# mandt-lab/PSLD

Hardware: AMD Instinct MI355X
Metric: train images/sec, CIFAR-10 PSLD (6ch 32x32) NCSN++ HSM step (higher is better)
Workload: dtype f32

## Files before the change

### include/psld_hip.h

```cpp
#ifndef PSLD_HIP_H
#define PSLD_HIP_H

#if defined(__HIP__) || defined(__HIPCC__)
#include <hip/hip_runtime_api.h>
#else
typedef struct ihipStream_t* hipStream_t;
#endif

#ifdef __cplusplus
extern "C" {
#endif


#define PSLD_ABI_VERSION 14
#define PSLD_COEFF_STRIDE 12

int psld_version(void);
const char* psld_last_error(void);

#define PSLD_MATH_F32 0
#define PSLD_MATH_BF16X6 1
#define PSLD_MATH_BF16X3 2
int psld_set_math_mode(int mode);
int psld_get_math_mode(void);
// ... 100 lines not shown
                           hipStream_t stream);
int psld_pack_frag_batch_x3(const long long* table_dev, int entries, long long total_items, hipStream_t stream);
int psld_gemm_split_x3_f32(const float* a1, int k1, const float* a2, int k2, int m, const void* bfrag, int n,
                           float* y, int ldy, const psld_epilogue_t* epi, hipStream_t stream);

int psld_attn_fwd_split_supported(int hw, int c);
int psld_attn_fwd_split_f32(const float* q, const float* k, const float* v, int ld, int batch, int hw, int c, float scale,
                            float* o, int ldo, float* p, hipStream_t stream);

int psld_conv3x3_wgrad_split_supported(int cout, int cin, int batch, int h, int w);
int psld_conv3x3_wgrad_split_cout_tile(int cout);
int psld_conv3x3_wgrad_split_f32(const float* dy, int lddy, int cout, const float* x, int cin,
                                 const float* x2, int cin2, int batch, int h, int w, float* slabs,
                                 int cin_total, int col0, int nsplit, hipStream_t stream);
int psld_conv3x3_wgrad_xlimb_f32(const float* dy, int lddy, int cout, const void* x_limb, int cin,
                                 const void* x2_limb, int cin2, int batch, int h, int w, float* slabs,
                                 int cin_total, int col0, int nsplit, hipStream_t stream);
int psld_conv3x3_wgrad_wino_supported(int cout, int cin, int cin2, int batch, int h, int w);
int psld_conv3x3_wgrad_wino_nsplit(int cout, int cin_total, int batch, int h, int w);
long long psld_conv3x3_wgrad_wino_ws_bytes(int cout, int cin_total, int nsplit);
int psld_conv3x3_wgrad_wino_f32(const float* dy, int lddy, int cout, const float* x, int cin, const float* x2, int cin2,
                                int batch, int h, int w, float* slabs, int nsplit, float* dw_oihw, int accumulate,
                                float alpha, hipStream_t stream);
int psld_gemm_tn_split_supported(int m, int n, int k);
int psld_gemm_tn_split_f32(int m, int n, int k, const float* a, int lda, const float* b, int ldb,
                           const float* b2, int ldb2, int n2, float* slabs, int ldc, int nsplit, hipStream_t stream);

int psld_bgemm_split_supported(int ta, int tb, int m, int n, int k);
int psld_bgemm_split_f32(int ta, int tb, int m, int n, int k, const float* a, int lda, long long stride_a,
                         const float* b, int ldb, long long stride_b, float* c, int ldc, long long stride_c,
                         int batch, float alpha, hipStream_t stream);

int psld_conv2d_wgrad_nhwc_f32(const float* dy, int lddy, int cout,
                               const float* x, int cin, int batch, int ih, int iw,
                               int kh, int kw, int stride, int pad, int oh, int ow,
                               float* slabs, int cin_total, int col0, int nsplit,
                               hipStream_t stream);

int psld_reduce_slabs_f32(const float* slabs, int nsplit, long long n, float* out,
                          int layout, int cout, int taps, int cin, float alpha, hipStream_t stream);

int psld_pack_oihw_to_ohwi_f32(const float* w, float* out, int cout, int cin, int taps, hipStream_t stream);
int psld_pack_oihw_to_dgrad_f32(const float* w, float* out, int cout, int cin, int taps, hipStream_t stream);

int psld_nchw_to_nhwc_f32(const float* x, float* y, int batch, int c, int hw, hipStream_t stream);
int psld_nhwc_to_nchw_f32(const float* x, float* y, int batch, int c, int hw, hipStream_t stream);
// ... 164 lines not shown
```

### psld_amd/_lib.py

```python
from __future__ import annotations

import ctypes as C
import os

_HERE = os.path.dirname(os.path.abspath(__file__))
LIB_PATH = os.environ.get("PSLD_HIP_LIB") or os.path.join(_HERE, "libpsld_hip.so")

c_f32p = C.c_void_p
c_f64p = C.c_void_p
c_stream = C.c_void_p
c_ll = C.c_longlong


class Epilogue(C.Structure):
    _fields_ = [
        ("alpha", C.c_float),
        ("bias", C.c_void_p),
        ("rowbias", C.c_void_p),
        ("ld_rowbias", C.c_int),
        ("rows_per_img", C.c_int),
        ("residual", C.c_void_p),
        ("ld_residual", C.c_int),
        ("residual_stride_batch", C.c_longlong),
        ("out_scale", C.c_float),
# ... 3 lines not shown
        ("gn_fine", C.c_int),
    ]


class SdeParams(C.Structure):
    _fields_ = [
        ("beta_0", C.c_double), ("beta_1", C.c_double), ("nu", C.c_double), ("gamma", C.c_double),
        ("m_inv", C.c_double), ("numerical_eps", C.c_double), ("decomp_lower", C.c_int),
    ]


class EmCoeffs(C.Structure):
    _fields_ = [
        ("beta", C.c_double), ("m_inv", C.c_double), ("gamma", C.c_double), ("nu", C.c_double),
        ("m", C.c_double),
        ("c11", C.c_float), ("c12", C.c_float), ("c21", C.c_float), ("c22", C.c_float),
        ("dt", C.c_double), ("score_mode", C.c_int), ("probability_flow", C.c_int),
    ]


class SscsCoeffs(C.Structure):
    _fields_ = [(n, C.c_double) for n in ("a_xx", "a_xm", "a_mx", "a_mm", "c11", "c12", "c21", "c22")]


I, F, D, LL, P = C.c_int, C.c_float, C.c_double, C.c_longlong, C.c_void_p
EP = C.POINTER(Epilogue)

ABI_VERSION = 14

SIGNATURES = {
    "psld_version": (I, []),
    "psld_last_error": (C.c_char_p, []),
    "psld_set_math_mode": (I, [I]),
    "psld_get_math_mode": (I, []),
    "psld_set_gn_bwd_kernel": (I, [I]),
    "psld_get_gn_bwd_kernel": (I, []),
    "psld_gemm_f32": (I, [I, I, I, I, I, P, I, LL, P, I, LL, P, I, LL, I, EP, P]),
    "psld_gemm_tn_splitk_f32": (I, [I, I, I, P, I, P, I, P, I, P]),
    "psld_conv2d_nhwc_f32": (I, [P, I, P, I, I, I, I, P, I, I, I, I, I, I, I, I, P, I, EP, P]),
    "psld_conv2d_workspace_bytes": (LL, [I, I, I, I]),
    "psld_conv2d_nhwc_ws_f32": (I, [P, I, P, I, I, I, I, P, I, I, I, I, I, I, I, I, P, I, EP, P, LL, P]),
    "psld_conv2d_wgrad_nhwc_f32": (I, [P, I, I, P, I, I, I, I, I, I, I, I, I, I, P, I, I, I, P]),
    "psld_conv3x3_frag_bytes": (LL, [I, I]),
    "psld_conv3x3_split_supported": (I, [I, I, I, I, I, I]),
    "psld_pack_conv3x3_frag": (I, [P, P, I, I, I, P]),
    "psld_pack_frag_batch": (I, [P, I, LL, P]),
# ... 18 lines not shown
    "psld_conv3x3_wino_gn_x3_f32": (I, [P, I, P, P, P, I, P, P, I, I, I, I, P, I, P, I, EP, P, LL, P]),
    "psld_gn_apply_limb_nhwc": (I, [P, P, P, P, I, I, I, I, F, C.c_ulonglong, P, P]),
    "psld_limb_bytes": (LL, [LL, I]),
    "psld_f32_to_limb": (I, [P, LL, I, P, P]),
    "psld_limb_to_f32": (I, [P, LL, I, P, P]),
    "psld_conv3x3_limb_f32": (I, [P, I, P, I, I, I, I, P, I, P, I, EP, P, LL, P]),
    "psld_gemm_frag_bytes": (LL, [I, I]),
    "psld_gemm_split_supported": (I, [I, I, I, I]),
    "psld_pack_gemm_frag": (I, [P, P, I, I, LL, LL, P]),
    "psld_gemm_split_f32": (I, [P, I, P, I, I, P, I, P, I, EP, P, LL, P]),
    "psld_gemm_frag_bytes_x3": (LL, [I, I]),
    "psld_gemm_split_x3_supported": (I, [I, I, I, I]),
    "psld_pack_gemm_frag_x3": (I, [P, P, I, I, LL, LL, P]),
    "psld_pack_frag_batch_x3": (I, [P, I, LL, P]),
    "psld_gemm_split_x3_f32": (I, [P, I, P, I, I, P, I, P, I, EP, P]),
    "psld_conv3x3_wgrad_split_supported": (I, [I, I, I, I, I]),
    "psld_conv3x3_wgrad_split_cout_tile": (I, [I]),
    "psld_conv3x3_wgrad_split_f32": (I, [P, I, I, P, I, P, I, I, I, I, P, I, I, I, P]),
    "psld_conv3x3_wgrad_xlimb_f32": (I, [P, I, I, P, I, P, I, I, I, I, P, I, I, I, P]),
    "psld_conv3x3_wgrad_wino_supported": (I, [I, I, I, I, I, I]),
    "psld_conv3x3_wgrad_wino_nsplit": (I, [I, I, I, I, I]),
    "psld_conv3x3_wgrad_wino_ws_bytes": (LL, [I, I, I]),
    "psld_conv3x3_wgrad_wino_f32": (I, [P, I, I, P, I, P, I, I, I, I, P, I, P, I, F, P]),
    "psld_gemm_tn_split_supported": (I, [I, I, I]),
    "psld_gemm_tn_split_f32": (I, [I, I, I, P, I, P, I, P, I, I, P, I, I, P]),
    "psld_bgemm_split_supported": (I, [I, I, I, I, I]),
    "psld_bgemm_split_f32": (I, [I, I, I, I, I, P, I, LL, P, I, LL, P, I, LL, I, F, P]),
    "psld_reduce_slabs_f32": (I, [P, I, LL, P, I, I, I, I, F, P]),
    "psld_pack_oihw_to_ohwi_f32": (I, [P, P, I, I, I, P]),
    "psld_pack_oihw_to_dgrad_f32": (I, [P, P, I, I, I, P]),
    "psld_nchw_to_nhwc_f32": (I, [P, P, I, I, I, P]),
    "psld_nhwc_to_nchw_f32": (I, [P, P, I, I, I, P]),
    "psld_gn_workspace_bytes": (LL, [I, I, I, I]),
    "psld_gn_stats_nhwc_f32": (I, [P, I, I, I, I, F, P, P, P, P, P, P, P, P]),
    "psld_gn_stats_from_partials_f32": (I, [P, I, I, I, I, I, F, P, P, P, P, P, P, P]),
    "psld_gn_apply_nhwc_f32": (I, [P, P, P, P, I, I, I, I, F, C.c_ulonglong, P, P]),
    "psld_gn_bwd_nhwc_f32": (I, [P, P, P, P, P, P, I, I, I, I, I, F, C.c_ulonglong, P, P, I, P, F, P, P, I, P, P]),
    "psld_gn_bwd_colsum_supported": (I, [I, I, I, I]),
    "psld_gn_bwd_team_rows": (I, [I, I, I, I]),
    "psld_gn_bwd_team_sync_bytes": (LL, []),
    "psld_gn_bwd_team_f32": (I, [P, P, P, P, P, P, I, I, I, I, I, F, C.c_ulonglong, P, P, I, P, F, P, P, I, P, P]),
    "psld_param_reduce2_f32": (I, [P, P, I, I, I, P, P, F, P]),
    "psld_param_reduce_batch_f32": (I, [P, I, I, P]),
    "psld_reduce_slabs_batch_units": (I, [LL, I, I, I]),
    "psld_reduce_slabs_batch_f32": (I, [P, I, LL, P]),
    "psld_upfirdn2d_f32": (I, [P, P, I, I, I, I, P, I, I, I, I, I, I, I, I, I, I, I, I, P]),
# ... 108 lines not shown
```

### psld_amd/csrc/wgrad_wino.hip

```cpp
#include "limb.h"
#include "psld_hip.h"
#include "tile_shared.h"

namespace {

typedef __attribute__((ext_vector_type(4))) short s16x4;
__device__ __forceinline__ u32x2 lds_tr16(const unsigned char* p) {
    const s16x4 v = __builtin_amdgcn_ds_read_tr16_b64_v4i16(
        (__attribute__((address_space(3))) s16x4*)(__attribute__((address_space(3))) void*)(p));
    return __builtin_bit_cast(u32x2, v);
}

constexpr int WW_CI = 128;
constexpr int WW_RSB = WW_CI * 2 + 32;
constexpr int WW_BLIMB = 32 * WW_RSB;
template <int CO>
struct WWGeom {
    static constexpr int RSA = CO * 2 + 32;
    static constexpr int ALIMB = 32 * RSA;
    static constexpr int IMG = 3 * (ALIMB + WW_BLIMB);
    static constexpr size_t LDS = 2 * (size_t)IMG;
    static constexpr int NY = CO / 32;
    static constexpr int CB = CO / 32;
};
// ... 42 lines not shown

template <int ABL = 0>
__device__ __forceinline__ void ww_store(unsigned char* d, int limb_stride, const f32x4& v) {
    unsigned h0, m0, l0, h1, m1, l1;
    if constexpr ((ABL & 1) != 0) {
        h0 = m0 = l0 = __float_as_uint(v[0]) ^ __float_as_uint(v[1]);
        h1 = m1 = l1 = __float_as_uint(v[2]) ^ __float_as_uint(v[3]);
    } else {
        ww_split3(v[0], v[1], h0, m0, l0);
        ww_split3(v[2], v[3], h1, m1, l1);
    }
    *reinterpret_cast<u32x2*>(d) = u32x2{h0, h1};
    *reinterpret_cast<u32x2*>(d + limb_stride) = u32x2{m0, m1};
    *reinterpret_cast<u32x2*>(d + 2 * limb_stride) = u32x2{l0, l1};
}

__device__ __forceinline__ f32x4 bload(const __amdgpu_buffer_rsrc_t& r, unsigned off) {
    return __builtin_bit_cast(f32x4, __builtin_amdgcn_raw_buffer_load_b128(r, off, 0, 0));
}
__device__ __forceinline__ __amdgpu_buffer_rsrc_t brsrc(const float* p) {
    return __builtin_amdgcn_make_buffer_rsrc(const_cast<float*>(p), 0, 0x7fffffff, 0x00020000);
}

template <int ABL = 0, int CO = 256, bool TAIL = false>
__global__ void __launch_bounds__(512) wwgrad_ws_kernel(const WWgradArgs a) {
    using G = WWGeom<CO>;
    constexpr int WW_CO = CO, WW_RSA = G::RSA, WW_ALIMB = G::ALIMB, WW_IMG = G::IMG, NY = G::NY, CB = G::CB;
    extern __shared__ __attribute__((aligned(16))) unsigned char smem[];
    const int tid = threadIdx.x;
    const int lane = tid & 63, wave = __builtin_amdgcn_readfirstlane(tid >> 6);

    const int units = 16 * a.cin_tiles * a.cout_tiles;
    const int vid = xcd_remap(blockIdx.x, gridDim.x);
    const int split = vid / units;
    int rest = vid - split * units;
    int pos = rest & 15;
    if constexpr (ABL != 0) {
        if (a.pos_override >= 0) pos = a.pos_override;
    }
    rest >>= 4;
    const int ci_tile = rest % a.cin_tiles, co_tile = rest / a.cin_tiles;
    const int pi = pos >> 2, pj = pos & 3;
    const int co0 = co_tile * WW_CO, ci_out = ci_tile * WW_CI;
    const int kt_beg = split * a.ktiles_per_split;
    const int nkt = min(a.ktiles_per_split, a.ktiles - kt_beg);

    if (wave >= 4) {
        const bool second = ci_out >= a.cin;
        const float* xsrc = second ? a.x2 : a.x;
        const int xc = second ? a.cin2 : a.cin;
        const int ci0 = second ? ci_out - a.cin : ci_out;
        const int pt = tid & 255;
        int xr1, xr2, xc1, xc2, yr1, ynr, yc1, ync;
        float xsr, xsc, ysr, ysc;
        x_combo(pi, xr1, xr2, xsr);
        x_combo(pj, xc1, xc2, xsc);
// ... 203 lines not shown
                for (int u = 0; u < 6; ++u)
#pragma unroll
                    for (int nb = 0; nb < 4; ++nb)
                        acc[cb][nb] = __builtin_amdgcn_mfma_f32_16x16x32_bf16(
                            __builtin_bit_cast(bf16x8, fa[cb & 1][PA[u]]), __builtin_bit_cast(bf16x8, fb[nb][PB[u]]), acc[cb][nb], 0, 0, 0);
            }
        }
        __syncthreads();
    }

    float* S = a.slabs + ((long long)split * 16 + pos) * a.cout * a.cin_total;
#pragma unroll
    for (int cb = 0; cb < CB; ++cb)
#pragma unroll
        for (int nb = 0; nb < 4; ++nb)
#pragma unroll
            for (int v = 0; v < 4; ++v) {
                const int co = co0 + wr * (CO / 2) + cb * 16 + 4 * g + v;
                if (!TAIL || (co < a.cout && ci_out + wc * 64 + nb * 16 + i16 < a.cin_total))
                    S[(long long)co * a.cin_total + ci_out + wc * 64 + nb * 16 + i16] = acc[cb][nb][v];
            }
}

__global__ void __launch_bounds__(64) wwgrad_reduce_kernel(const float* __restrict__ slabs, int nsplit, long long n, float* __restrict__ dw,
                                                           int accumulate, float alpha) {
    const long long idx = (long long)blockIdx.x * 64 + threadIdx.x;
    if (idx >= n) return;
    float m[16];
#pragma unroll
    for (int p = 0; p < 16; ++p) m[p] = 0.f;
    const float* src = slabs + idx;
    for (int sp = 0; sp < nsplit; ++sp) {
        float v[16];
#pragma unroll
        for (int p = 0; p < 16; ++p) v[p] = __builtin_nontemporal_load(src + ((long long)sp * 16 + p) * n);
#pragma unroll
        for (int p = 0; p < 16; ++p) m[p] += v[p];
    }
    float t[4][3];
#pragma unroll
    for (int i = 0; i < 4; ++i) {
        const float h = 0.5f * (m[4 * i + 1] + m[4 * i + 2]), d = 0.5f * (m[4 * i + 1] - m[4 * i + 2]);
        t[i][0] = m[4 * i] + h;
        t[i][1] = d;
        t[i][2] = h - m[4 * i + 3];
    }
    float o[9];
#pragma unroll
    for (int kx = 0; kx < 3; ++kx) {
        const float h = 0.5f * (t[1][kx] + t[2][kx]), d = 0.5f * (t[1][kx] - t[2][kx]);
        o[kx] = t[0][kx] + h;
        o[3 + kx] = d;
        o[6 + kx] = h - t[3][kx];
    }
    float* out = dw + idx * 9;
#pragma unroll
    for (int e = 0; e < 9; ++e) out[e] = accumulate ? out[e] + alpha * o[e] : alpha * o[e];
}

inline int ww_co_tile(int cout) { return cout % 256 ? 128 : 256; }

int ilog2(int v) {
    int l = 0;
    while ((1 << l) < v) ++l;
    return l;
}

}

static bool ww_width_ok(int c) { return c >= 128 && c % 32 == 0; }

extern "C" int psld_conv3x3_wgrad_wino_supported(int cout, int cin, int cin2, int batch, int h, int w) {
    if (batch <= 0 || cin2 < 0 || !ww_width_ok(cout) || !ww_width_ok(cin) || (cin2 && (cin % WW_CI || !ww_width_ok(cin2)))) return 0;
    if (h != w || !(w == 8 || w == 16 || w == 32 || w == 64 || w == 128)) return 0;
    return ((long long)batch * h * w / 4) % 32 == 0;
}

extern "C" int psld_conv3x3_wgrad_wino_nsplit(int cout, int cin_total, int batch, int h, int w) {
    if (!ww_width_ok(cout) || !ww_width_ok(cin_total)) return 0;
    const int units = 16 * (int)cdiv(cout, ww_co_tile(cout)) * (int)cdiv(cin_total, WW_CI);
    const long long ktiles = (long long)batch * h * w / 4 / 32;
    static int cus[PSLD_MAX_DEVICES] = {};
    int& n = cus[psld_device_slot()];
    if (n == 0) {
        int dev = 0;
        if (hipGetDevice(&dev) != hipSuccess || hipDeviceGetAttribute(&n, hipDeviceAttributeMultiprocessorCount, dev) != hipSuccess || n <= 0) n = 256;
    }
    int ns = n / units;
    if (ns < 1) ns = 1;
    if (ns > ktiles) ns = (int)ktiles;
    const long long per = (ktiles + ns - 1) / ns;
    return (int)((ktiles + per - 1) / per);
}

extern "C" long long psld_conv3x3_wgrad_wino_ws_bytes(int cout, int cin_total, int nsplit) {
    return (long long)nsplit * 16 * cout * cin_total * 4;
}

extern "C" int psld_conv3x3_wgrad_wino_f32(const float* dy, int lddy, int cout, const float* x, int cin, const float* x2, int cin2,
                                           int batch, int h, int w, float* slabs, int nsplit, float* dw_oihw, int accumulate,
                                           float alpha, hipStream_t stream) {
    PSLD_CHECK_ARG(dy && x && slabs && dw_oihw && nsplit >= 1 && (cin2 == 0 || x2), "psld_conv3x3_wgrad_wino_f32: bad args");
    PSLD_CHECK_ARG(psld_conv3x3_wgrad_wino_supported(cout, cin, cin2, batch, h, w),
                   "psld_conv3x3_wgrad_wino_f32: unsupported shape cout=%d cin=%d+%d B=%d %dx%d", cout, cin, cin2, batch, h, w);
    PSLD_CHECK_ARG(aligned16(dy) && aligned16(x) && (cin2 == 0 || aligned16(x2)) && lddy % 4 == 0 && lddy >= cout,
                   "psld_conv3x3_wgrad_wino_f32: unaligned operand");
    const long long ktiles = (long long)batch * h * w / 4 / 32;
    const long long per_split = (ktiles + nsplit - 1) / nsplit;
    PSLD_CHECK_ARG((ktiles + per_split - 1) / per_split == nsplit, "psld_conv3x3_wgrad_wino_f32: %d splits of %lld K tiles leave empty slabs", nsplit, ktiles);
    WWgradArgs a{};
    a.dy = dy; a.lddy = lddy; a.x = x; a.cin = cin; a.x2 = x2; a.cin2 = cin2;
    a.H = h; a.W = w;
    const int tw = w / 2 < 32 ? w / 2 : 32;
    a.lg_tw = ilog2(tw); a.tw_mask = tw - 1; a.th_mask = h / 2 - 1;
    a.rows_per_kt = 32 >> a.lg_tw;
    a.lg_kpr = ilog2(w / 2 / tw); a.kpr_mask = w / 2 / tw - 1;
    const int co_tile = ww_co_tile(cout);
    a.cout_tiles = (int)cdiv(cout, co_tile); a.cin_tiles = (int)cdiv(cin + cin2, WW_CI);
    const bool tail = cout % co_tile || (cin + cin2) % WW_CI;
    a.ktiles = (int)ktiles; a.ktiles_per_split = (int)per_split;
    a.slabs = slabs; a.cout = cout; a.cin_total = cin + cin2;
    a.pos_override = -1;
    const dim3 grid((unsigned)(16 * a.cout_tiles * a.cin_tiles * nsplit));
#ifdef PSLD_ABLATIONS
    static const int abl = [] { const char* v = getenv("PSLD_WWGRAD_ABL"); return v ? atoi(v) : 0; }();
    static const int pos_ov = [] { const char* v = getenv("PSLD_WWGRAD_POS"); return v ? atoi(v) : -1; }();
    a.pos_override = pos_ov;
#define WW_ABL_CASE(N)                                                                                                              \
    case N:                                                                                                                         \
        (void)hipFuncSetAttribute(reinterpret_cast<const void*>(&wwgrad_ws_kernel<N, 256>), hipFuncAttributeMaxDynamicSharedMemorySize, (int)WWGeom<256>::LDS); \
        hipLaunchKernelGGL((wwgrad_ws_kernel<N, 256>), grid, dim3(512), WWGeom<256>::LDS, stream, a);                                \
        PSLD_CHECK_LAUNCH("wwgrad_ws_kernel (ablation)");                                                                           \
        launched = true;                                                                                                            \
        break;
    bool launched = false;
    switch (co_tile == 256 && !tail ? abl : 0) {
        WW_ABL_CASE(1) WW_ABL_CASE(2) WW_ABL_CASE(3) WW_ABL_CASE(4) WW_ABL_CASE(8) WW_ABL_CASE(12) WW_ABL_CASE(16) WW_ABL_CASE(32) WW_ABL_CASE(64)
        default: break;
    }
#undef WW_ABL_CASE
    if (!launched)
#endif
    {
    static PsldPerDeviceFlag configured_; bool& configured = configured_.here();
    if (!configured) {
// ... 5 lines not shown
        if (e == hipSuccess)
            e = hipFuncSetAttribute(reinterpret_cast<const void*>(&wwgrad_ws_kernel<0, 256, true>), hipFuncAttributeMaxDynamicSharedMemorySize, (int)WWGeom<256>::LDS);
        if (e != hipSuccess) {
            psld_set_error("psld_conv3x3_wgrad_wino_f32: hipFuncSetAttribute failed: %s", hipGetErrorString(e));
            return PSLD_ERR_LAUNCH;
        }
        configured = true;
    }
    if (tail && co_tile == 256)
        hipLaunchKernelGGL((wwgrad_ws_kernel<0, 256, true>), grid, dim3(512), WWGeom<256>::LDS, stream, a);
    else if (tail)
        hipLaunchKernelGGL((wwgrad_ws_kernel<0, 128, true>), grid, dim3(512), WWGeom<128>::LDS, stream, a);
    else if (co_tile == 256)
        hipLaunchKernelGGL((wwgrad_ws_kernel<0, 256>), grid, dim3(512), WWGeom<256>::LDS, stream, a);
    else
        hipLaunchKernelGGL((wwgrad_ws_kernel<0, 128>), grid, dim3(512), WWGeom<128>::LDS, stream, a);
    PSLD_CHECK_LAUNCH("wwgrad_ws_kernel");
    }
    const long long n = (long long)cout * a.cin_total;
    hipLaunchKernelGGL(wwgrad_reduce_kernel, dim3((unsigned)cdiv(n, 64)), dim3(64), 0, stream, slabs, nsplit, n, dw_oihw, accumulate, alpha);
    PSLD_CHECK_LAUNCH("wwgrad_reduce_kernel");
    return PSLD_OK;
}
```

### psld_amd/ops.py

```python
from __future__ import annotations

import ctypes as C
import functools
import os
from typing import Optional, Sequence, Tuple

import numpy as np
import torch

from . import _lib
from ._lib import Epilogue, EmCoeffs, SdeParams, SscsCoeffs, check

Tensor = torch.Tensor
INV_SQRT2 = float(1.0 / np.sqrt(2.0))


def lib():
    return _lib.load()


_stream_cache = []


def _stream() -> int:
# ... 478 lines not shown


@functools.lru_cache(maxsize=None)
def conv3x3_wgrad_wino_plan(cout: int, cin_total: int, b: int, h: int, w: int):
    ns = int(lib().psld_conv3x3_wgrad_wino_nsplit(cout, cin_total, b, h, w))
    return ns, int(lib().psld_conv3x3_wgrad_wino_ws_bytes(cout, cin_total, ns))


def conv3x3_wgrad_wino(dy: Tensor, cout: int, x: Tensor, dw: Tensor, x2: Optional[Tensor] = None, accumulate: bool = False,
                       slabs: Optional[Tensor] = None, nsplit: Optional[int] = None, alpha: float = 1.0):
    b, h, w, cin = x.shape
    cin2 = x2.shape[-1] if x2 is not None else 0
    ns, wsb = conv3x3_wgrad_wino_plan(cout, cin + cin2, b, h, w)
    if nsplit is not None:
        ns, wsb = nsplit, int(lib().psld_conv3x3_wgrad_wino_ws_bytes(cout, cin + cin2, nsplit))
    if slabs is None:
        slabs = workspace(wsb, x.device)
    assert slabs.numel() * slabs.element_size() >= wsb and dw.is_contiguous() and dw.numel() == cout * (cin + cin2) * 9
    check(lib().psld_conv3x3_wgrad_wino_f32(dy.data_ptr(), cout, cout, x.data_ptr(), cin, _p(x2), cin2, b, h, w,
                                            slabs.data_ptr(), ns, dw.data_ptr(), 1 if accumulate else 0, float(alpha), _stream()),
          "psld_conv3x3_wgrad_wino_f32")


def conv2d_wgrad_nhwc(dy: Tensor, cout: int, x: Tensor, kh: int, kw: int, stride: int, pad: int, oh: int, ow: int,
                      slabs: Tensor, cin_total: int, col0: int, nsplit: int):
    b, ih, iw, cin = x.shape
    check(lib().psld_conv2d_wgrad_nhwc_f32(dy.data_ptr(), cout, cout, x.data_ptr(), cin, b, ih, iw, kh, kw, stride,
                                           pad, oh, ow, slabs.data_ptr(), cin_total, col0, nsplit, _stream()),
          "psld_conv2d_wgrad_nhwc_f32")


def reduce_slabs(slabs: Tensor, nsplit: int, n: int, out: Tensor, layout: int = 0, cout: int = 0, taps: int = 0,
                 cin: int = 0, alpha: float = 1.0):
    check(lib().psld_reduce_slabs_f32(slabs.data_ptr(), nsplit, n, out.data_ptr(), layout, cout, taps, cin, alpha,
                                      _stream()), "psld_reduce_slabs_f32")


def pack_ohwi(w_oihw: Tensor, out: Tensor):
    co, ci = w_oihw.shape[0], w_oihw.shape[1]
    taps = w_oihw.shape[2] * w_oihw.shape[3]
    check(lib().psld_pack_oihw_to_ohwi_f32(w_oihw.data_ptr(), out.data_ptr(), co, ci, taps, _stream()), "pack_ohwi")


def pack_dgrad(w_oihw: Tensor, out: Tensor):
    co, ci = w_oihw.shape[0], w_oihw.shape[1]
    taps = w_oihw.shape[2] * w_oihw.shape[3]
# ... 677 lines not shown
```

### psld_amd/score_fn.py

```python
from __future__ import annotations

import functools
import math
from typing import List, Optional

import numpy as np
import torch
import torch.nn as nn

from . import ops
from .registry import register_module
from .weight_cache import Entry, WeightCache

Tensor = torch.Tensor
_ALIGN = 64


def default_init(shape, scale: float = 1.0) -> Tensor:
    scale = 1e-10 if scale == 0 else scale
    rf = float(np.prod(shape)) / shape[1] / shape[0]
    fan_in, fan_out = shape[1] * rf, shape[0] * rf
    variance = scale / ((fan_in + fan_out) / 2)
    return (torch.rand(*shape) * 2.0 - 1.0) * math.sqrt(3 * variance)

# ... 87 lines not shown
        self.gp = gp
        self.used = False
        self.want_gsum = want_gsum
        self.gsum = None


class _CatNode:
    __slots__ = ("a", "b")

    def __init__(self, a: _Node, b: _Node):
        self.a = a
        self.b = b


_OVERLAP_MAX_PIXELS = 65536
_SLAB_FLUSH_BYTES = 1 << 30


def _gbuf(node: _Node):
    if node.g is None:
        node.g = torch.empty_like(node.v)
        return node.g, False
    return node.g, True


_RESIDENT_BLOCKS = 512


@functools.lru_cache(maxsize=None)
def _pick_nsplit(tiles: int, k: int, min_k: int = 256, resident: int = _RESIDENT_BLOCKS) -> int:
    max_split = max(1, k // min_k)
    best, best_eff = 1, 0.0
    for ns in range(1, min(max_split, 128) + 1):
        blocks = tiles * ns
        rounds = -(-blocks // resident)
        eff = blocks / (rounds * resident)
        if eff > best_eff + 0.02:
            best, best_eff = ns, eff
    return best


def _fir_kernel(k) -> np.ndarray:
    k = np.asarray(k, dtype=np.float32)
    k = np.outer(k, k)
    k /= np.sum(k)
    return k
# ... 19 lines not shown
        p = self.k_down.shape[0] - 2
        self.pad_up = ((p + 1) // 2 + 1, p // 2)
        self.pad_down = ((p + 1) // 2, p // 2)
        self.temb_act: Optional[_Node] = None
        self.watermark = None
        self.side = None
        self.side_queue = []
        self.side_group = net.side_group
        self.want_dx = False
        mode = ops.math_mode()
        self.split = mode in ("bf16x6", "bf16x3")
        self.x3 = mode == "bf16x3" and not record
        import os as _os
        self.limb_planes = _os.environ.get("PSLD_LIMB_PLANES", "1") != "0"
        self.fused_attn = _os.environ.get("PSLD_FUSED_ATTN", "1") != "0"
        self.gn_bwd_colsum = _os.environ.get("PSLD_GN_BWD_COLSUM", "1") == "1"
        self.dx_nchw = None
        self.defer = bool(net.defer_param_grads) and record
        self.dense_batched = False
        self.dense_ok = False
        self.dense_pending = []
        self.pjobs, self.pblocks = [], 0
        self.sjobs, self.sitems, self.sbytes = [], 0, 0

    def push(self, fn, module=None):
        if self.tape is not None:
            self.tape.append((fn, module))

    def g(self, p: nn.Parameter) -> Tensor:
        return self.net._grad_view(p)

    def on_side(self, fn, *tensors):
        if self.side is None:
            fn()
            return
        self.side_queue.append((fn, tensors))
        if len(self.side_queue) >= self.side_group:
            self.flush_side()

    def flush_side(self):
        if not self.side_queue:
            return
        queue, self.side_queue = self.side_queue, []
        ev = torch.cuda.Event()
        cur = torch.cuda.current_stream()
        ev.record(cur)
# ... 41 lines not shown
            return ops.workspace(nbytes, device)
        return self.net._slab_arena().alloc(nbytes)

    def reduce_slabs(self, slabs: Tensor, nsplit: int, n: int, out: Tensor, layout: int = 0, cout: int = 1, taps: int = 1,
                     cin: int = 1, alpha: float = 1.0, more: bool = False):
        units = ops.slab_units(n, layout, taps, cin) if self.defer else 0
        if units == 0 or out.data_ptr() % 16:
            ops.reduce_slabs(slabs, nsplit, n, out, layout=layout, cout=cout, taps=taps, cin=cin, alpha=alpha)
            return
        self.sjobs.append(ops.slab_job(slabs, nsplit, n, out, layout, taps, cin, alpha) + (self.sitems, units))
        self.sitems += units
        self.sbytes += 4 * n * nsplit
        if self.sbytes >= _SLAB_FLUSH_BYTES and not more:
            self.flush_slabs()

    def flush_slabs(self):
        if self.sjobs:
            jobs, items = self.sjobs, self.sitems
            self.sjobs, self.sitems, self.sbytes = [], 0, 0
            rows = [v for job in jobs for v in job]
            table = self.net._tables.get(rows, self.net._params()[0].device)
            ops.reduce_slabs_batch(table, len(jobs), items, sum(4 * j[2] * (j[1] + 1) for j in jobs))
            self.net._slab_arena().reset()

    def flush_dense(self):
        pend, self.dense_pending = self.dense_pending, []
        if not pend:
            return
        net, dtp_all, act = self.net, self.dtp_all, self.temb_act.v
        b, total = dtp_all.shape
        kd = act.shape[1]
        lo, hi = min(o for o, _, _ in pend), max(o + c for o, c, _ in pend)
        if hi - lo == sum(c for _, c, _ in pend) and lo % 4 == 0 and ops.gemm_tn_split_supported(hi - lo, kd, b):
            dwcat = net._persist("dwcat", (total, kd))
            ops.gemm_tn_split(hi - lo, kd, b, dtp_all[:, lo:hi], total, act, kd, dwcat[lo:hi], kd, 1)
            rows, first = [], 0
            for o, c, d0 in pend:
                n4 = c * kd // 4
                rows += [dwcat.data_ptr() + 4 * o * kd, self.g(d0.weight).data_ptr(), n4, first]
                first += n4
            ops.copy_batch(net._tables.get(rows, dwcat.device), len(pend), first)
        else:
            for o, c, d0 in pend:
                if o % 4 == 0 and ops.gemm_tn_split_supported(c, kd, b):
                    ops.gemm_tn_split(c, kd, b, dtp_all[:, o:o + c], total, act, kd, self.g(d0.weight), kd, 1)
                else:
                    ops.gemm_raw(1, 0, c, kd, b, dtp_all[:, o:o + c], total, 0, act, kd, 0, self.g(d0.weight), kd, 0)

    def flush_deferred(self):
        self.on_side(self.flush_slabs)
        self.flush_params()
        self.flush_dense()

    def finish_backward(self):
        if self.defer:
            self.flush_deferred()
        self.join_side()

    def gn_backward(self, dy: Tensor, x: Tensor, st, gamma: Tensor, beta: Tensor, dgamma: Tensor, dbeta: Tensor, act: bool,
                    dx: Tensor, accumulate_dx: bool = False, add: Optional[Tensor] = None, add_scale: float = 1.0,
                    drop_p: float = 0.0, seed: int = 0, seed_dev=None, groups: Optional[int] = None,
                    colsum_img: Optional[Tensor] = None, ld_img: int = 0, last_writer_of: Optional[_Node] = None):
        b, h, w, c = x.shape
        pa = self.net._param_arena()
        node = last_writer_of
        k = ops.gn_bwd_team_wanted(b, h * w, c, groups, add is not None or accumulate_dx) if colsum_img is None else 0
        fold = node is not None and node.want_gsum and colsum_img is None and self.gn_bwd_colsum and \
            (k > 0 or ops.gn_bwd_colsum_supported(b, h * w, c, groups))
        rows = b * max(k, 1)
        sums = pa.floats(rows, 2, c)
        if fold:
            colsum_img, ld_img = pa.floats(rows, c), c
# ... 9 lines not shown
        if fold:
            node.gsum = colsum_img

    def bias_from(self, node: _Node, dout: Tensor, bias: nn.Parameter, alpha: float = 1.0,
                  bias2: Optional[nn.Parameter] = None) -> bool:
        gsum, node.gsum = node.gsum, None
        if gsum is not None:
            self.defer_param(gsum, gsum.shape[0], gsum.shape[1], gsum.shape[1], self.g(bias),
                             self.g(bias2) if bias2 is not None else None, alpha)
            return True
        return False

    def wgrad(self, dy: Tensor, x: Tensor, conv: _Affine, k: int, stride: int, pad: int, alpha: float = 1.0,
              x2: Optional[Tensor] = None):
        b, oh, ow, cout = dy.shape
        c1 = x.shape[-1]
        c2 = x2.shape[-1] if x2 is not None else 0
        cin = c1 + c2
        taps = k * k
        n = cout * taps * cin
        assert x2 is None or self.split, "two-source weight gradients exist on the limb kernels only"
        if self.split and k == 3 and stride == 1 and pad == 1 and not isinstance(x, ops.LimbPlanes) and \
                ops.conv3x3_wgrad_wino_wanted(cout, c1, c2, b, oh, ow):
            ops.conv3x3_wgrad_wino(dy, cout, x, self.g(conv.weight), x2=x2, alpha=alpha)
            return
        if self.split and k == 3 and stride == 1 and pad == 1 and \
                ops.conv3x3_wgrad_split_supported(cout, c1, b, oh, ow) and \
                (x2 is None or ops.conv3x3_wgrad_split_supported(cout, c2, b, oh, ow)):
            ktiles = b * oh * ow // 32
            co_tile = ops.conv3x3_wgrad_split_cout_tile(cout)
            resident = 768 if co_tile == 64 else (512 if isinstance(x, ops.LimbPlanes) else 256)
            nsplit = _pick_nsplit((cout // co_tile) * (cin // 64) * 3, ktiles * 32, min_k=128, resident=resident)
            per = -(-ktiles // nsplit)
            nsplit = -(-ktiles // per)
            slabs = self.slabs_for(4 * n * nsplit, dy.device)
            ops.conv3x3_wgrad_split(dy, cout, x, slabs, cin, 0, nsplit, x2)
            self.reduce_slabs(slabs, nsplit, n, self.g(conv.weight), layout=1, cout=cout, taps=taps, cin=cin, alpha=alpha)
            return
        if self.split and k == 1 and stride == 1 and pad == 0 and ops.gemm_tn_split_supported(cout, c1, b * oh * ow) and \
                c2 % 128 == 0:
            nsplit = self._tn_split(cout, cin, b * oh * ow)
            slabs = self.slabs_for(4 * n * nsplit, dy.device)
            ops.gemm_tn_split(cout, c1, b * oh * ow, dy, cout, x, c1, slabs, cin, nsplit, x2, c2, c2)
            self.reduce_slabs(slabs, nsplit, n, self.g(conv.weight), alpha=alpha)
            return
        assert x2 is None, "unsupported two-source weight gradient"
# ... 1461 lines not shown
```

Before: 1260.

## Batch small Winograd weight-gradient convolutions into grouped multi-job launches

Adds a grouped Winograd 3x3 weight-gradient path. Several small deferred wgrad jobs are parked and then run in one multi-job kernel plus one multi-job reduce kernel, with a planner that picks per-job split counts so the combined work groups fill the device's compute units. The aim is to cut launch overhead and the under-occupancy of small low-resolution convolutions. In exchange it adds deferral and bookkeeping, a larger slab workspace, and a dependency on the flush ordering of the deferred gradients.

```diff
diff --git a/include/psld_hip.h b/include/psld_hip.h
--- a/include/psld_hip.h
+++ b/include/psld_hip.h
@@ -146,6 +146,20 @@
 int psld_conv3x3_wgrad_wino_f32(const float* dy, int lddy, int cout, const float* x, int cin, const float* x2, int cin2,
                                 int batch, int h, int w, float* slabs, int nsplit, float* dw_oihw, int accumulate,
                                 float alpha, hipStream_t stream);
+#define PSLD_WGRAD_GROUP_MAX 8
+typedef struct psld_wgrad_wino_job {
+    const float* dy;
+    const float* x;
+    const float* x2;
+    float* dw_oihw;
+    int lddy, cout, cin, cin2, batch, h, w;
+    int nsplit;
+    int accumulate;
+    float alpha;
+} psld_wgrad_wino_job_t;
+int psld_conv3x3_wgrad_wino_group_supported(int cout, int cin, int cin2, int batch, int h, int w);
+int psld_conv3x3_wgrad_wino_group_plan(const int* shapes, int* nsplit_out, long long* slab_bytes_out, int njobs, int cus);
+int psld_conv3x3_wgrad_wino_group_f32(const psld_wgrad_wino_job_t* jobs, int njobs, float* slabs, hipStream_t stream);
 int psld_gemm_tn_split_supported(int m, int n, int k);
 int psld_gemm_tn_split_f32(int m, int n, int k, const float* a, int lda, const float* b, int ldb,
                            const float* b2, int ldb2, int n2, float* slabs, int ldc, int nsplit, hipStream_t stream);
diff --git a/psld_amd/_lib.py b/psld_amd/_lib.py
--- a/psld_amd/_lib.py
+++ b/psld_amd/_lib.py
@@ -49,6 +49,16 @@
 class SscsCoeffs(C.Structure):
     _fields_ = [(n, C.c_double) for n in ("a_xx", "a_xm", "a_mx", "a_mm", "c11", "c12", "c21", "c22")]
 
+
+class WgradWinoJob(C.Structure):
+    _fields_ = [
+        ("dy", C.c_void_p), ("x", C.c_void_p), ("x2", C.c_void_p), ("dw_oihw", C.c_void_p),
+        ("lddy", C.c_int), ("cout", C.c_int), ("cin", C.c_int), ("cin2", C.c_int), ("batch", C.c_int),
+        ("h", C.c_int), ("w", C.c_int), ("nsplit", C.c_int), ("accumulate", C.c_int), ("alpha", C.c_float),
+    ]
+
+
+WGRAD_GROUP_MAX = 8
 
 I, F, D, LL, P = C.c_int, C.c_float, C.c_double, C.c_longlong, C.c_void_p
 EP = C.POINTER(Epilogue)
@@ -113,6 +123,9 @@
     "psld_conv3x3_wgrad_wino_nsplit": (I, [I, I, I, I, I]),
     "psld_conv3x3_wgrad_wino_ws_bytes": (LL, [I, I, I]),
     "psld_conv3x3_wgrad_wino_f32": (I, [P, I, I, P, I, P, I, I, I, I, P, I, P, I, F, P]),
+    "psld_conv3x3_wgrad_wino_group_supported": (I, [I, I, I, I, I, I]),
+    "psld_conv3x3_wgrad_wino_group_plan": (I, [C.POINTER(I), C.POINTER(I), C.POINTER(LL), I, I]),
+    "psld_conv3x3_wgrad_wino_group_f32": (I, [C.POINTER(WgradWinoJob), I, P, P]),
     "psld_gemm_tn_split_supported": (I, [I, I, I]),
     "psld_gemm_tn_split_f32": (I, [I, I, I, P, I, P, I, P, I, I, P, I, I, P]),
     "psld_bgemm_split_supported": (I, [I, I, I, I, I]),
diff --git a/psld_amd/csrc/wgrad_wino.hip b/psld_amd/csrc/wgrad_wino.hip
--- a/psld_amd/csrc/wgrad_wino.hip
+++ b/psld_amd/csrc/wgrad_wino.hip
@@ -88,8 +88,8 @@
     return __builtin_amdgcn_make_buffer_rsrc(const_cast<float*>(p), 0, 0x7fffffff, 0x00020000);
 }
 
-template <int ABL = 0, int CO = 256, bool TAIL = false>
-__global__ void __launch_bounds__(512) wwgrad_ws_kernel(const WWgradArgs a) {
+template <int ABL, int CO, bool TAIL>
+__device__ __forceinline__ void wwgrad_ws_body(const WWgradArgs a, const int vid) {
     using G = WWGeom<CO>;
     constexpr int WW_CO = CO, WW_RSA = G::RSA, WW_ALIMB = G::ALIMB, WW_IMG = G::IMG, NY = G::NY, CB = G::CB;
     extern __shared__ __attribute__((aligned(16))) unsigned char smem[];
@@ -97,7 +97,6 @@
     const int lane = tid & 63, wave = __builtin_amdgcn_readfirstlane(tid >> 6);
 
     const int units = 16 * a.cin_tiles * a.cout_tiles;
-    const int vid = xcd_remap(blockIdx.x, gridDim.x);
     const int split = vid / units;
     int rest = vid - split * units;
     int pos = rest & 15;
@@ -347,9 +346,30 @@
             }
 }
 
-__global__ void __launch_bounds__(64) wwgrad_reduce_kernel(const float* __restrict__ slabs, int nsplit, long long n, float* __restrict__ dw,
-                                                           int accumulate, float alpha) {
-    const long long idx = (long long)blockIdx.x * 64 + threadIdx.x;
+template <int ABL = 0, int CO = 256, bool TAIL = false>
+__global__ void __launch_bounds__(512) wwgrad_ws_kernel(const WWgradArgs a) {
+    wwgrad_ws_body<ABL, CO, TAIL>(a, xcd_remap(blockIdx.x, gridDim.x));
+}
+
+constexpr int WW_GROUP_MAX = PSLD_WGRAD_GROUP_MAX;
+struct WWMultiArgs {
+    WWgradArgs job[WW_GROUP_MAX];
+    int first[WW_GROUP_MAX + 1];
+    int njobs;
+};
+template <int CO = 256, bool TAIL = false>
+__global__ void __launch_bounds__(512) wwgrad_ws_multi_kernel(const WWMultiArgs m) {
+    const int vid = xcd_remap(blockIdx.x, gridDim.x);
+    if (vid >= m.first[m.njobs]) return;
+    int j = 0;
+#pragma unroll
+    for (int i = 1; i < WW_GROUP_MAX; ++i) j += (i < m.njobs && vid >= m.first[i]) ? 1 : 0;
+    j = __builtin_amdgcn_readfirstlane(j);
+    wwgrad_ws_body<0, CO, TAIL>(m.job[j], vid - m.first[j]);
+}
+
+__device__ __forceinline__ void wwgrad_reduce_body(const float* __restrict__ slabs, int nsplit, long long n, float* __restrict__ dw,
+                                                   int accumulate, float alpha, const long long idx) {
     if (idx >= n) return;
     float m[16];
 #pragma unroll
@@ -383,6 +403,31 @@
     for (int e = 0; e < 9; ++e) out[e] = accumulate ? out[e] + alpha * o[e] : alpha * o[e];
 }
 
+__global__ void __launch_bounds__(64) wwgrad_reduce_kernel(const float* __restrict__ slabs, int nsplit, long long n, float* __restrict__ dw,
+                                                           int accumulate, float alpha) {
+    wwgrad_reduce_body(slabs, nsplit, n, dw, accumulate, alpha, (long long)blockIdx.x * 64 + threadIdx.x);
+}
+
+struct WWReduceJob {
+    const float* slabs;
+    float* dw;
+    long long n;
+    int nsplit, accumulate;
+    float alpha;
+    int first;
+};
+struct WWReduceMultiArgs {
+    WWReduceJob job[WW_GROUP_MAX];
+    int njobs;
+};
+__global__ void __launch_bounds__(64) wwgrad_reduce_multi_kernel(const WWReduceMultiArgs m) {
+    int j = 0;
+#pragma unroll
+    for (int i = 1; i < WW_GROUP_MAX; ++i) j += (i < m.njobs && (int)blockIdx.x >= m.job[i].first) ? 1 : 0;
+    const WWReduceJob& r = m.job[j];
+    wwgrad_reduce_body(r.slabs, r.nsplit, r.n, r.dw, r.accumulate, r.alpha, (long long)((int)blockIdx.x - r.first) * 64 + threadIdx.x);
+}
+
 inline int ww_co_tile(int cout) { return cout % 256 ? 128 : 256; }
 
 int ilog2(int v) {
@@ -395,23 +440,44 @@
 
 static bool ww_width_ok(int c) { return c >= 128 && c % 32 == 0; }
 
+static WWgradArgs ww_fill_args(const float* dy, int lddy, int cout, const float* x, int cin, const float* x2, int cin2, int h, int w,
+                               long long ktiles, long long per_split, float* slabs) {
+    WWgradArgs a{};
+    a.dy = dy; a.lddy = lddy; a.x = x; a.cin = cin; a.x2 = x2; a.cin2 = cin2;
+    a.H = h; a.W = w;
+    const int tw = w / 2 < 32 ? w / 2 : 32;
+    a.lg_tw = ilog2(tw); a.tw_mask = tw - 1; a.th_mask = h / 2 - 1;
+    a.rows_per_kt = 32 >> a.lg_tw;
+    a.lg_kpr = ilog2(w / 2 / tw); a.kpr_mask = w / 2 / tw - 1;
+    const int co_tile = ww_co_tile(cout);
+    a.cout_tiles = (int)cdiv(cout, co_tile); a.cin_tiles = (int)cdiv(cin + cin2, WW_CI);
+    a.ktiles = (int)ktiles; a.ktiles_per_split = (int)per_split;
+    a.slabs = slabs; a.cout = cout; a.cin_total = cin + cin2;
+    a.pos_override = -1;
+    return a;
+}
+
 extern "C" int psld_conv3x3_wgrad_wino_supported(int cout, int cin, int cin2, int batch, int h, int w) {
     if (batch <= 0 || cin2 < 0 || !ww_width_ok(cout) || !ww_width_ok(cin) || (cin2 && (cin % WW_CI || !ww_width_ok(cin2)))) return 0;
     if (h != w || !(w == 8 || w == 16 || w == 32 || w == 64 || w == 128)) return 0;
     return ((long long)batch * h * w / 4) % 32 == 0;
 }
 
-extern "C" int psld_conv3x3_wgrad_wino_nsplit(int cout, int cin_total, int batch, int h, int w) {
-    if (!ww_width_ok(cout) || !ww_width_ok(cin_total)) return 0;
-    const int units = 16 * (int)cdiv(cout, ww_co_tile(cout)) * (int)cdiv(cin_total, WW_CI);
-    const long long ktiles = (long long)batch * h * w / 4 / 32;
+static int ww_device_cus() {
     static int cus[PSLD_MAX_DEVICES] = {};
     int& n = cus[psld_device_slot()];
     if (n == 0) {
         int dev = 0;
         if (hipGetDevice(&dev) != hipSuccess || hipDeviceGetAttribute(&n, hipDeviceAttributeMultiprocessorCount, dev) != hipSuccess || n <= 0) n = 256;
     }
-    int ns = n / units;
+    return n;
+}
+
+extern "C" int psld_conv3x3_wgrad_wino_nsplit(int cout, int cin_total, int batch, int h, int w) {
+    if (!ww_width_ok(cout) || !ww_width_ok(cin_total)) return 0;
+    const int units = 16 * (int)cdiv(cout, ww_co_tile(cout)) * (int)cdiv(cin_total, WW_CI);
+    const long long ktiles = (long long)batch * h * w / 4 / 32;
+    int ns = ww_device_cus() / units;
     if (ns < 1) ns = 1;
     if (ns > ktiles) ns = (int)ktiles;
     const long long per = (ktiles + ns - 1) / ns;
@@ -433,19 +499,9 @@
     const long long ktiles = (long long)batch * h * w / 4 / 32;
     const long long per_split = (ktiles + nsplit - 1) / nsplit;
     PSLD_CHECK_ARG((ktiles + per_split - 1) / per_split == nsplit, "psld_conv3x3_wgrad_wino_f32: %d splits of %lld K tiles leave empty slabs", nsplit, ktiles);
-    WWgradArgs a{};
-    a.dy = dy; a.lddy = lddy; a.x = x; a.cin = cin; a.x2 = x2; a.cin2 = cin2;
-    a.H = h; a.W = w;
-    const int tw = w / 2 < 32 ? w / 2 : 32;
-    a.lg_tw = ilog2(tw); a.tw_mask = tw - 1; a.th_mask = h / 2 - 1;
-    a.rows_per_kt = 32 >> a.lg_tw;
-    a.lg_kpr = ilog2(w / 2 / tw); a.kpr_mask = w / 2 / tw - 1;
+    const WWgradArgs a = ww_fill_args(dy, lddy, cout, x, cin, x2, cin2, h, w, ktiles, per_split, slabs);
     const int co_tile = ww_co_tile(cout);
-    a.cout_tiles = (int)cdiv(cout, co_tile); a.cin_tiles = (int)cdiv(cin + cin2, WW_CI);
     const bool tail = cout % co_tile || (cin + cin2) % WW_CI;
-    a.ktiles = (int)ktiles; a.ktiles_per_split = (int)per_split;
-    a.slabs = slabs; a.cout = cout; a.cin_total = cin + cin2;
-    a.pos_override = -1;
     const dim3 grid((unsigned)(16 * a.cout_tiles * a.cin_tiles * nsplit));
 #ifdef PSLD_ABLATIONS
     static const int abl = [] { const char* v = getenv("PSLD_WWGRAD_ABL"); return v ? atoi(v) : 0; }();
@@ -497,3 +553,83 @@
     PSLD_CHECK_LAUNCH("wwgrad_reduce_kernel");
     return PSLD_OK;
 }
+
+extern "C" int psld_conv3x3_wgrad_wino_group_supported(int cout, int cin, int cin2, int batch, int h, int w) {
+    return psld_conv3x3_wgrad_wino_supported(cout, cin, cin2, batch, h, w) && cout % 256 == 0 && cin % WW_CI == 0 && cin2 % WW_CI == 0;
+}
+
+extern "C" int psld_conv3x3_wgrad_wino_group_plan(const int* shapes, int* nsplit_out, long long* slab_bytes_out, int njobs, int cus) {
+    if (!shapes || !nsplit_out || njobs < 1 || njobs > WW_GROUP_MAX) return 0;
+    if (cus <= 0) cus = ww_device_cus();
+    long long units[WW_GROUP_MAX], kt[WW_GROUP_MAX], max_kt = 0, sum_units = 0;
+    for (int j = 0; j < njobs; ++j) {
+        const int* s = shapes + 5 * j;
+        if (!psld_conv3x3_wgrad_wino_group_supported(s[0], s[1], 0, s[2], s[3], s[4])) return 0;
+        units[j] = 16LL * (s[0] / 256) * (s[1] / WW_CI);
+        kt[j] = (long long)s[2] * s[3] * s[4] / 4 / 32;
+        sum_units += units[j];
+        if (kt[j] > max_kt) max_kt = kt[j];
+    }
+    if (sum_units > cus) return 0;
+    long long P = max_kt;
+    for (long long p = 1; p < max_kt; ++p) {
+        long long wgs = 0;
+        for (int j = 0; j < njobs; ++j) wgs += units[j] * cdiv(kt[j], p);
+        if (wgs <= cus) { P = p; break; }
+    }
+    long long total = 0, bytes = 0;
+    for (int j = 0; j < njobs; ++j) {
+        const long long per = cdiv(kt[j], cdiv(kt[j], P));
+        const int ns = (int)cdiv(kt[j], per);
+        nsplit_out[j] = ns;
+        total += units[j] * ns;
+        bytes += psld_conv3x3_wgrad_wino_ws_bytes(shapes[5 * j], shapes[5 * j + 1], ns);
+    }
+    if (slab_bytes_out) *slab_bytes_out = bytes;
+    return (int)total;
+}
+
+extern "C" int psld_conv3x3_wgrad_wino_group_f32(const psld_wgrad_wino_job_t* jobs, int njobs, float* slabs, hipStream_t stream) {
+    PSLD_CHECK_ARG(jobs && slabs && njobs >= 1 && njobs <= WW_GROUP_MAX, "psld_conv3x3_wgrad_wino_group_f32: bad args (1..%d jobs)", WW_GROUP_MAX);
+    PSLD_CHECK_ARG(aligned16(slabs), "psld_conv3x3_wgrad_wino_group_f32: unaligned workspace");
+    WWMultiArgs m{};
+    WWReduceMultiArgs r{};
+    m.njobs = r.njobs = njobs;
+    long long first = 0, rfirst = 0;
+    float* S = slabs;
+    for (int j = 0; j < njobs; ++j) {
+        const psld_wgrad_wino_job_t& q = jobs[j];
+        PSLD_CHECK_ARG(q.dy && q.x && q.dw_oihw && q.nsplit >= 1 && (q.cin2 == 0 || q.x2), "psld_conv3x3_wgrad_wino_group_f32: job %d: bad args", j);
+        PSLD_CHECK_ARG(psld_conv3x3_wgrad_wino_group_supported(q.cout, q.cin, q.cin2, q.batch, q.h, q.w),
+                       "psld_conv3x3_wgrad_wino_group_f32: job %d: unsupported shape cout=%d cin=%d+%d B=%d %dx%d", j, q.cout, q.cin, q.cin2, q.batch, q.h, q.w);
+        PSLD_CHECK_ARG(aligned16(q.dy) && aligned16(q.x) && (q.cin2 == 0 || aligned16(q.x2)) && q.lddy % 4 == 0 && q.lddy >= q.cout,
+                       "psld_conv3x3_wgrad_wino_group_f32: job %d: unaligned operand", j);
+        const long long ktiles = (long long)q.batch * q.h * q.w / 4 / 32;
+        const long long per_split = (ktiles + q.nsplit - 1) / q.nsplit;
+        PSLD_CHECK_ARG((ktiles + per_split - 1) / per_split == q.nsplit, "psld_conv3x3_wgrad_wino_group_f32: job %d: %d splits of %lld K tiles leave empty slabs", j, q.nsplit, ktiles);
+        m.job[j] = ww_fill_args(q.dy, q.lddy, q.cout, q.x, q.cin, q.cin2 ? q.x2 : nullptr, q.cin2, q.h, q.w, ktiles, per_split, S);
+        m.first[j] = (int)first;
+        first += 16LL * m.job[j].cout_tiles * m.job[j].cin_tiles * q.nsplit;
+        const long long n = (long long)q.cout * (q.cin + q.cin2);
+        r.job[j] = WWReduceJob{S, q.dw_oihw, n, q.nsplit, q.accumulate, q.alpha, (int)rfirst};
+        rfirst += cdiv(n, 64);
+        S += (long long)q.nsplit * 16 * n;
+        PSLD_CHECK_ARG(first < (1LL << 24) && rfirst < (1LL << 30), "psld_conv3x3_wgrad_wino_group_f32: group too large");
+    }
+    for (int j = njobs; j <= WW_GROUP_MAX; ++j) m.first[j] = (int)first;
+    static PsldPerDeviceFlag configured_; bool& configured = configured_.here();
+    if (!configured) {
+        const hipError_t e = hipFuncSetAttribute(reinterpret_cast<const void*>(&wwgrad_ws_multi_kernel<256, false>), hipFuncAttributeMaxDynamicSharedMemorySize, (int)WWGeom<256>::LDS);
+        if (e != hipSuccess) {
+            psld_set_error("psld_conv3x3_wgrad_wino_group_f32: hipFuncSetAttribute failed: %s", hipGetErrorString(e));
+            return PSLD_ERR_LAUNCH;
+        }
+        configured = true;
+    }
+    const long long q16 = cdiv(cdiv(first, 8), 16) * 16;
+    hipLaunchKernelGGL((wwgrad_ws_multi_kernel<256, false>), dim3((unsigned)(8 * q16)), dim3(512), WWGeom<256>::LDS, stream, m);
+    PSLD_CHECK_LAUNCH("wwgrad_ws_multi_kernel");
+    hipLaunchKernelGGL(wwgrad_reduce_multi_kernel, dim3((unsigned)rfirst), dim3(64), 0, stream, r);
+    PSLD_CHECK_LAUNCH("wwgrad_reduce_multi_kernel");
+    return PSLD_OK;
+}
diff --git a/psld_amd/ops.py b/psld_amd/ops.py
--- a/psld_amd/ops.py
+++ b/psld_amd/ops.py
@@ -524,6 +524,71 @@
           "psld_conv3x3_wgrad_wino_f32")
 
 
+WGRAD_GROUP_MAX = _lib.WGRAD_GROUP_MAX
+_WGRAD_GROUP_BELOW = 16
+_WGRAD_GROUP_K = 64
+_WGRAD_GROUP_MODE: Optional[int] = None
+
+
+def set_wgrad_group(mode: Optional[int]):
+    global _WGRAD_GROUP_MODE
+    assert mode in (None, 0, 2)
+    _WGRAD_GROUP_MODE = mode
+
+
+def wgrad_group_mode() -> int:
+    return 1 if _WGRAD_GROUP_MODE is None else _WGRAD_GROUP_MODE
+
+
+@functools.lru_cache(maxsize=None)
+def conv3x3_wgrad_wino_group_supported(cout: int, cin: int, cin2: int, b: int, h: int, w: int) -> bool:
+    return bool(lib().psld_conv3x3_wgrad_wino_group_supported(cout, cin, cin2, b, h, w))
+
+
+@functools.lru_cache(maxsize=None)
+def conv3x3_wgrad_wino_group_wanted(cout: int, cin: int, cin2: int, b: int, h: int, w: int) -> bool:
+    if not conv3x3_wgrad_wino_group_supported(cout, cin, cin2, b, h, w):
+        return False
+    ns, _ = conv3x3_wgrad_wino_plan(cout, cin + cin2, b, h, w)
+    return -(-(b * h * w // 128) // ns) <= _WGRAD_GROUP_BELOW
+
+
+@functools.lru_cache(maxsize=None)
+def conv3x3_wgrad_wino_group_plan(shapes: Tuple[Tuple[int, int, int, int, int], ...], cus: int = 0):
+    n = len(shapes)
+    flat = (C.c_int * (5 * n))(*[v for s in shapes for v in s])
+    ns = (C.c_int * max(n, 1))()
+    nbytes = C.c_longlong(0)
+    wgs = int(lib().psld_conv3x3_wgrad_wino_group_plan(flat, ns, C.byref(nbytes), n, cus))
+    return wgs, tuple(ns[:n]) if wgs else (), int(nbytes.value) if wgs else 0
+
+
+@functools.lru_cache(maxsize=None)
+def conv3x3_wgrad_wino_group_nsplit(cout: int, cin_total: int, b: int, h: int, w: int, cus: int) -> int:
+    shape = (cout, cin_total, b, h, w)
+    if not conv3x3_wgrad_wino_group_supported(cout, cin_total, 0, b, h, w):
+        return 0
+    at_target = 16 * (cout // 256) * (cin_total // 128) * -(-(b * h * w // 128) // _WGRAD_GROUP_K)
+    n = min(max(cus // at_target, 1), WGRAD_GROUP_MAX)
+    wgs, ns, _ = conv3x3_wgrad_wino_group_plan((shape,) * n, cus)
+    return ns[0] if wgs else 0
+
+
+def conv3x3_wgrad_wino_group(jobs: Sequence[tuple]):
+    arr = (_lib.WgradWinoJob * len(jobs))()
+    wsb = 0
+    for q, (dy, cout, x, x2, dw, accumulate, alpha, nsplit) in zip(arr, jobs):
+        b, h, w, cin = x.shape
+        cin2 = x2.shape[-1] if x2 is not None else 0
+        assert dw.is_contiguous() and dw.numel() == cout * (cin + cin2) * 9
+        q.dy, q.x, q.x2, q.dw_oihw = dy.data_ptr(), x.data_ptr(), _p(x2), dw.data_ptr()
+        q.lddy, q.cout, q.cin, q.cin2, q.batch, q.h, q.w = cout, cout, cin, cin2, b, h, w
+        q.nsplit, q.accumulate, q.alpha = nsplit, 1 if accumulate else 0, float(alpha)
+        wsb += 64 * nsplit * cout * (cin + cin2)
+    slabs = workspace(wsb, jobs[0][0].device)
+    check(lib().psld_conv3x3_wgrad_wino_group_f32(arr, len(jobs), slabs.data_ptr(), _stream()), "psld_conv3x3_wgrad_wino_group_f32")
+
+
 def conv2d_wgrad_nhwc(dy: Tensor, cout: int, x: Tensor, kh: int, kw: int, stride: int, pad: int, oh: int, ow: int,
                       slabs: Tensor, cin_total: int, col0: int, nsplit: int):
     b, ih, iw, cin = x.shape
diff --git a/psld_amd/score_fn.py b/psld_amd/score_fn.py
--- a/psld_amd/score_fn.py
+++ b/psld_amd/score_fn.py
@@ -133,6 +133,11 @@
         node.g = torch.empty_like(node.v)
         return node.g, False
     return node.g, True
+
+
+@functools.lru_cache(maxsize=None)
+def _compute_units(device) -> int:
+    return int(torch.cuda.get_device_properties(device).multi_processor_count)
 
 
 _RESIDENT_BLOCKS = 512
@@ -198,6 +203,7 @@
         self.dense_pending = []
         self.pjobs, self.pblocks = [], 0
         self.sjobs, self.sitems, self.sbytes = [], 0, 0
+        self.wjobs, self.wunits = [], 0
 
     def push(self, fn, module=None):
         if self.tape is not None:
@@ -285,6 +291,29 @@
             table = self.net._tables.get(rows, self.net._params()[0].device)
             ops.reduce_slabs_batch(table, len(jobs), items, sum(4 * j[2] * (j[1] + 1) for j in jobs))
             self.net._slab_arena().reset()
+
+    def park_wgrad(self, dy: Tensor, x: Tensor, x2: Optional[Tensor], conv: _Affine, alpha: float) -> bool:
+        b, h, w, cout = dy.shape
+        cin = x.shape[-1] + (x2.shape[-1] if x2 is not None else 0)
+        cus = _compute_units(dy.device)
+        nsplit = ops.conv3x3_wgrad_wino_group_nsplit(cout, cin, b, h, w, cus)
+        if nsplit == 0:
+            return False
+        units = 16 * (cout // 256) * (cin // 128) * nsplit
+        if ops.wgrad_group_mode() == 2:
+            nsplit = ops.conv3x3_wgrad_wino_plan(cout, cin, b, h, w)[0]
+        if self.wjobs and self.wunits + units > cus:
+            self.flush_wgroup()
+        self.wjobs.append((dy, cout, x, x2, self.g(conv.weight), False, alpha, nsplit))
+        self.wunits += units
+        if self.wunits >= cus or len(self.wjobs) == ops.WGRAD_GROUP_MAX:
+            self.flush_wgroup()
+        return True
+
+    def flush_wgroup(self):
+        jobs, self.wjobs, self.wunits = self.wjobs, [], 0
+        if jobs:
+            ops.conv3x3_wgrad_wino_group(jobs)
 
     def flush_dense(self):
         pend, self.dense_pending = self.dense_pending, []
@@ -311,6 +340,7 @@
                     ops.gemm_raw(1, 0, c, kd, b, dtp_all[:, o:o + c], total, 0, act, kd, 0, self.g(d0.weight), kd, 0)
 
     def flush_deferred(self):
+        self.on_side(self.flush_wgroup)
         self.on_side(self.flush_slabs)
         self.flush_params()
         self.flush_dense()
@@ -366,6 +396,9 @@
         assert x2 is None or self.split, "two-source weight gradients exist on the limb kernels only"
         if self.split and k == 3 and stride == 1 and pad == 1 and not isinstance(x, ops.LimbPlanes) and \
                 ops.conv3x3_wgrad_wino_wanted(cout, c1, c2, b, oh, ow):
+            if self.defer and ops.wgrad_group_mode() != 0 and ops.conv3x3_wgrad_wino_group_wanted(cout, c1, c2, b, oh, ow) and \
+                    self.park_wgrad(dy, x, x2, conv, alpha):
+                return
             ops.conv3x3_wgrad_wino(dy, cout, x, self.g(conv.weight), x2=x2, alpha=alpha)
             return
         if self.split and k == 3 and stride == 1 and pad == 1 and \
```

Result: no change. 1268 (median of 6 runs) (+0.6%).
